# mache102/HashNeRF-pytorch

Measured on AMD Instinct MI355X. Metric: training rays/sec (fwd+bwd) on chair; PSNR@5k iters, higher is better.
Workload: dtype fp32 (MLP GEMMs split-bf16 MFMA: 3 parts fwd, 2 parts grads); 1 GPU; chair 1xMI355X N_rand=4096 64+128 L16 F2 T19 finest512 (BASELINE configs[1]); rays_per_gpu=4096, global_batch=4096, samples_per_ray=64+128, log2_hashmap_size=19, finest_res=512, parallelism=dp1

## Files before the change

hashnerf-pytorch_amd/_lib.py:

```python
from __future__ import annotations

import ctypes as C
import os
from typing import Optional

import torch

HERE = os.path.dirname(os.path.abspath(__file__))
LIB_PATH = os.environ.get("HN_LIB_PATH") or os.path.join(HERE, "lib", "libhashnerf_amd.so")
MAX_LEVELS = 32
ABI_VERSION = 14
RENDER_FEAT_PER_RAY = 9728
MLP_PARAMS = 9344
MLP_PACKED_FLOATS = 30208

_lib = None


class HnGrid(C.Structure):
    _fields_ = [("n_levels", C.c_int32), ("n_features", C.c_int32),
                ("log2_hashmap_size", C.c_int32), ("reserved", C.c_int32),
                ("box_min", C.c_float * 3), ("box_max", C.c_float * 3),
                ("grid_size", (C.c_float * 3) * MAX_LEVELS)]

# ... 28 lines not shown
                ("rgb0", _P), ("depth0", _P), ("acc0", _P), ("sparsity0", _P),
                ("z_std", _P), ("z_coarse", _P), ("z_fine", _P), ("raw_c", _P), ("raw_f", _P),
                ("fine_src", _P), ("feat", _P), ("weights_packed", C.c_int32), ("skip_dead_color", C.c_int32),
                ("loss", C.POINTER(HnRenderLoss))]


class HnImageArgs(C.Structure):
    _fields_ = [("n_views", C.c_int32), ("H", C.c_int32), ("W", C.c_int32), ("pose_stride", C.c_int32),
                ("fx", C.c_float), ("fy", C.c_float), ("cx", C.c_float), ("cy", C.c_float),
                ("near", C.c_float), ("far", C.c_float), ("poses", _P), ("t_vals", _P), ("u", _P), ("table", _P),
                ("coarse", HnMlp), ("fine", HnMlp), ("rgb", _P), ("depth", _P), ("acc", _P), ("rays", _P),
                ("weights_packed", C.c_int32)]


IMAGE_VARIANTS = {"reencode": 1, "row_major": 2}


class HnRadamTensor(C.Structure):
    _fields_ = [("p", _P), ("g", _P), ("m", _P), ("v", _P), ("n", C.c_int64),
                ("beta1", C.c_float), ("beta2", C.c_float), ("one_minus_beta1", C.c_float),
                ("one_minus_beta2", C.c_float), ("eps", C.c_float), ("neg_wd_lr", C.c_float),
                ("neg_step_lr", C.c_float), ("mode", C.c_int32), ("has_wd", C.c_int32),
                ("reserved", C.c_int32)]


class HnRaySampler(C.Structure):
    _fields_ = [("H", C.c_int32), ("W", C.c_int32), ("crop_y0", C.c_int32), ("crop_x0", C.c_int32),
                ("crop_h", C.c_int32), ("crop_w", C.c_int32), ("fx", C.c_float), ("fy", C.c_float),
                ("cx", C.c_float), ("cy", C.c_float), ("near", C.c_float), ("far", C.c_float),
                ("seed", C.c_uint64)]
# ... 70 lines not shown
    "hn_sample_pool": (C.c_int32, [C.POINTER(HnRayPool), _P, _P, _P, C.c_int64, C.c_int64, _P, _P, _P]),
    "hn_sample_pool_ordered": (C.c_int32, [C.POINTER(HnRayPool), _P, _P, _P, C.c_int64, C.c_int64,
                                           C.POINTER(C.c_float), C.POINTER(C.c_float), _P, _P, _P, C.c_uint64,
                                           C.POINTER(HnUniformDraw), C.c_int32, _P]),
    "hn_blender_images": (C.c_int32, [_P, C.c_int64, C.c_int32, C.c_int32, C.c_int32, C.c_int32, _P, _P]),
    "hn_loss_fwd": (C.c_int32, [_P, _P, _P, _P, _P, C.c_int64, _P, C.c_int32, C.c_float, C.c_float,
                                C.c_float, _P, _P]),
    "hn_loss_bwd": (C.c_int32, [_P, _P, _P, C.c_int64, C.c_int32, C.c_float, C.c_float, C.c_float, _P,
                                _P, _P, _P, _P, _P, _P]),
    "hn_loss_fwd_bwd": (C.c_int32, [_P, _P, _P, _P, _P, C.c_int64, _P, C.c_int32, C.c_float, C.c_float,
                                    C.c_float, _P, _P, _P, _P, _P, _P, _P, _P]),
    "hn_render_workspace_bytes": (C.c_size_t, [C.POINTER(HnRenderCfg), C.c_int64]),
    "hn_render_scatter_mode": (C.c_int32, [C.POINTER(HnRenderCfg), C.c_int64]),
    "hn_render_fwd": (C.c_int32, [C.POINTER(HnRenderCfg), C.POINTER(HnRenderFwdArgs), _P,
                                  C.c_size_t, _P]),
    "hn_render_bwd": (C.c_int32, [C.POINTER(HnRenderCfg), C.POINTER(HnRenderBwdArgs), _P,
                                  C.c_size_t, _P]),
    "hn_render_image_workspace_bytes": (C.c_size_t, [C.POINTER(HnRenderCfg)]),
    "hn_render_image": (C.c_int32, [C.POINTER(HnRenderCfg), C.POINTER(HnImageArgs), _P, C.c_size_t, _P]),
    "hn_render_image_variant": (C.c_int32, [C.POINTER(HnRenderCfg), C.POINTER(HnImageArgs), C.c_int32, _P,
                                            C.c_size_t, _P]),
    "hn_render_bins": (C.c_int32, [C.POINTER(HnRenderCfg), C.c_int64, C.POINTER(C.c_int32)]),
    "hn_render_bwd_owner": (C.c_int32, [C.POINTER(HnRenderCfg), C.POINTER(HnRenderBwdArgs), _P,
                                        C.c_size_t, C.c_int32, C.c_int32, _P]),
}


def lib():
    global _lib
    if _lib is None:
# ... 85 lines not shown
```

hashnerf-pytorch_amd/csrc/hn_mlp.h:

```cpp
#pragma once
#include "hn_common.h"

namespace hn {

constexpr int kSplitF = 3;
constexpr int kSplitB = 2;
enum : int { R_F0, R_F1, R_F2G, R_F2S, R_F3, R_F4, R_B4, R_B3, R_B2G, R_B2S, R_B1, R_B0, R_N };
constexpr int kRegKS[R_N] = {16, 32, 8, 8, 32, 32, 4, 32, 32, 32, 8, 32};
constexpr int kRegOB[R_N] = {2, 1, 2, 2, 2, 1, 2, 2, 1, 1, 2, 1};
constexpr int kSplitFC = kSplitF;
constexpr int reg_ns(int r) {
  return kRegKS[r] % 8 ? 0 : (r < R_F2G ? kSplitF : (r < R_B4 ? kSplitFC : kSplitB));
}
constexpr int reg_gpo(int r) { return reg_ns(r) ? reg_ns(r) * kRegKS[r] / 8 : kRegKS[r] / 4; }
constexpr int reg_off(int r) {
  int o = 0;
  for (int i = 0; i < r; ++i) o += kRegOB[i] * reg_gpo(i) * 256;
  return o;
}
enum : int {
  G_F0 = reg_off(R_F0), G_F1 = reg_off(R_F1), G_F2G = reg_off(R_F2G), G_F2S = reg_off(R_F2S),
  G_F3 = reg_off(R_F3), G_F4 = reg_off(R_F4), G_B4 = reg_off(R_B4), G_B3 = reg_off(R_B3),
  G_B2G = reg_off(R_B2G), G_B2S = reg_off(R_B2S), G_B1 = reg_off(R_B1), G_B0 = reg_off(R_B0),
  G_END = reg_off(R_N)
};
static_assert(G_END <= HN_MLP_PACKED_FLOATS, "packed size");

enum : int { W_S0 = 0, W_S1 = 2048, W_C0 = 3072, W_C1 = 5056, W_C2 = 9152, W_END = 9344 };
static_assert(W_END == HN_MLP_PARAMS, "param count");

struct FragGlobal {
  static constexpr bool kRing = false;
  const float* P;
  HN_DEV f32x4 operator()(int off, int lane) const { return frag_load(P, off, lane); }
};
struct FwdChunk {
  int r, ob, c;
};
constexpr FwdChunk kFwdSeq[] = {
    {R_F0, 0, 0}, {R_F0, 0, 1}, {R_F0, 1, 0}, {R_F0, 1, 1}, {R_F1, 0, 0}, {R_F1, 0, 1}, {R_F1, 0, 2},
    {R_F1, 0, 3}, {R_F2G, 0, 0}, {R_F2G, 1, 0}, {R_F3, 0, 0}, {R_F3, 0, 1}, {R_F3, 0, 2}, {R_F3, 0, 3},
    {R_F3, 1, 0}, {R_F3, 1, 1}, {R_F3, 1, 2}, {R_F3, 1, 3}, {R_F4, 0, 0}, {R_F4, 0, 1}, {R_F4, 0, 2},
    {R_F4, 0, 3}};
constexpr int kFwdSeqN = sizeof(kFwdSeq) / sizeof(kFwdSeq[0]);
constexpr int fwd_chunk_off(const FwdChunk& q) { return reg_off(q.r) + (q.ob * reg_gpo(q.r) + reg_ns(q.r) * q.c) * 256; }
constexpr int fwd_next_off(int r, int ob, int c) {
  for (int i = 0; i < kFwdSeqN; ++i)
    if (kFwdSeq[i].r == r && kFwdSeq[i].ob == ob && kFwdSeq[i].c == c) return fwd_chunk_off(kFwdSeq[(i + 1) % kFwdSeqN]);
  return -1;
}
struct FragRing {
  static constexpr bool kRing = true;
  const float* P;
  float* slot;
  HN_DEV f32x4 operator()(int off, int lane) const { return frag_load(P, off, lane); }
};
HN_DEV void ring_fill(const float* P, float* slot, int off, int lane) {
  int so = off * 4;
  asm volatile("" : "+s"(so));
  const __amdgpu_buffer_rsrc_t rs =
      __builtin_amdgcn_make_buffer_rsrc(const_cast<float*>(opaque_ptr(P)), (short)0, 0x7fffffff, 0x00020000);
#pragma unroll
  for (int q = 0; q < 3; ++q)
    __builtin_amdgcn_raw_ptr_buffer_load_lds(rs, (__attribute__((address_space(3))) void*)(slot + 256 * q), 16,
                                             lane * 16, so + 1024 * q, 0, 0);
}
HN_DEV void fwd_ring_start(const float* P, float* slot, int lane) {
  ring_fill(P, slot, fwd_chunk_off(kFwdSeq[0]), lane);
}
template <int R, typename BF, typename Src>
HN_DEV f32x16 gemm_src(const Src& src, int ob, f32x16 acc, int lane, BF bval);
template <int R, typename BF>
HN_DEV f32x16 gemm(const float* __restrict__ P, int ob, f32x16 acc, int lane, BF bval) {
  return gemm_src<R>(FragGlobal{P}, ob, acc, lane, bval);
}
template <int R, typename BF, typename Src>
HN_DEV f32x16 gemm_src(const Src& src, int ob, f32x16 acc, int lane, BF bval) {
  constexpr int KS = kRegKS[R], NS = reg_ns(R), GPO = reg_gpo(R), OFF = reg_off(R);
  auto ld = [&](int g) { return src(OFF + (ob * GPO + g) * 256, lane); };
  if constexpr (NS > 0) {
#pragma unroll
    for (int c = 0; c < KS / 8; ++c) {
      SP<NS> a;
      if constexpr (Src::kRing && NS == 3) {
        asm volatile("s_waitcnt vmcnt(0)" ::: "memory");
#pragma unroll
        for (int q = 0; q < NS; ++q) a.p[q] = as_bf16x8(*reinterpret_cast<const f32x4*>(src.slot + 256 * q + 4 * lane));
        asm volatile("s_waitcnt lgkmcnt(0)" ::: "memory");
        ring_fill(src.P, src.slot, fwd_next_off(R, ob, c), lane);
      } else {
#pragma unroll
        for (int q = 0; q < NS; ++q) a.p[q] = as_bf16x8(ld(NS * c + q));
      }
      const SP<NS> b = splitn<NS>([&](int j) { return bval(8 * c + j); });
// ... 295 lines not shown
```

hashnerf-pytorch_amd/csrc/hn_render.hip:

```cpp
#include "hn_render_args.h"
#include "hn_render_fwd.h"
#include "hn_render_image.h"
#include "hn_mlp_bwd.h"
#include "hn_bwd_binned.h"
#include "hn_bwd_atomic.h"

#include <math.h>

namespace hn {

__global__ __launch_bounds__(256) void render_comp_bwd_kernel(B1K k) {
  __shared__ float lds[kFwdWaves][kSf * 5];
  const int wave = __builtin_amdgcn_readfirstlane((int)threadIdx.x >> 6);
  const int lane = threadIdx.x & 63;
  if (k.bins && blockIdx.x == 0) zero_ovf_book(k);
  if (k.lout && blockIdx.x == 0) {
    loss_fwd_block<64 * kFwdWaves>(k.lrgb, k.lrgb0, k.ltarget, k.lsp, k.lsp0, k.B, k.ltv, k.n_tv, k.lworld,
                                   k.lsparse_w, k.ltv_w, k.lout);
    return;
  }
  const int64_t w = (int64_t)(blockIdx.x - (k.lout ? 1 : 0)) * kFwdWaves + wave;
  __shared__ unsigned long long cmask[kFwdWaves / 2];
  const bool active = w < 2 * k.B;
  uint32_t nzf = 0u;
// ... 236 lines not shown
  return bwd_plan(cfg, n_rays).bytes();
}

extern "C" int32_t hn_render_scatter_mode(const hn_render_cfg* cfg, int64_t n_rays) {
  return bwd_mode(cfg, n_rays) == kModeSplit ? 2 : 1;
}

extern "C" int32_t hn_device_faults(int32_t* faults, int32_t clear) {
  if (!faults) return HN_E_NULL;
  int32_t st = hip_status(hipMemcpyFromSymbol(faults, HIP_SYMBOL(g_hn_fault), sizeof(int32_t)));
  if (st || !clear || *faults == 0) return st;
  const int32_t zero = 0;
  return hip_status(hipMemcpyToSymbol(HIP_SYMBOL(g_hn_fault), &zero, sizeof(int32_t)));
}

extern "C" int32_t hn_render_fwd(const hn_render_cfg* cfg, const hn_render_fwd_args* a,
                                 void* workspace, size_t ws_bytes, void* stream) {
  int32_t st = check_cfg(cfg);
  if (st) return st;
  if (!a) return HN_E_NULL;
  if (a->n_rays < 0) return HN_E_SHAPE;
  if (a->n_rays == 0) return HN_OK;
  if (!a->rays || !a->t_vals || !a->u || !a->table || !mlp_ok(a->coarse) || !mlp_ok(a->fine))
    return HN_E_NULL;
  if (cfg->perturb && !a->t_rand) return HN_E_NULL;
  if (!a->rgb || !a->depth || !a->acc || !a->sparsity || !a->rgb0 || !a->depth0 || !a->acc0 ||
      !a->sparsity0 || !a->z_std || !a->z_coarse || !a->z_fine || !a->raw_c || !a->raw_f ||
      !a->fine_src)
    return HN_E_NULL;
  if (!workspace) return HN_E_NULL;
  const BwdPlan plan = bwd_plan(cfg, a->n_rays);
  if (ws_bytes < plan.bytes()) return HN_E_WORKSPACE;
  const bool ni64 = cfg->n_importance == kNi64;
  if (ni64 && a->feat && plan.mode != kModeSplit) return HN_E_SHAPE;
// ... 9 lines not shown
  k.perturb = cfg->perturb;
  k.B = a->n_rays;
  k.rays = a->rays; k.t_rand = a->t_rand;
  k.noise_c = a->noise_c; k.noise_f = a->noise_f;
  k.rgb = a->rgb; k.depth = a->depth; k.acc = a->acc; k.sparsity = a->sparsity;
  k.rgb0 = a->rgb0; k.depth0 = a->depth0; k.acc0 = a->acc0; k.sparsity0 = a->sparsity0;
  k.z_std = a->z_std; k.z_coarse = a->z_coarse; k.z_fine = a->z_fine;
  k.raw_c = a->raw_c; k.raw_f = a->raw_f; k.fine_src = a->fine_src; k.feat = a->feat;
  k.feat_nt = cfg->grid.log2_hashmap_size > 20;
  k.skip_dead = a->skip_dead_color != 0;
  k.ltarget = nullptr;
  k.lgm = k.lsparse = 0.f;
  k.draw = nullptr;
  k.uflags = nullptr;
  k.stamp = nullptr;
  const unsigned blocks = (unsigned)((a->n_rays + kFwdBlockWaves - 1) / kFwdBlockWaves);
  if (a->loss) {
    const WsDraw w = ws_draw(workspace, a->n_rays);
    k.ltarget = a->loss->target;
    k.lgm = (1.f / a->loss->world) / (float)(3 * a->n_rays);
    k.lsparse = 1.f * a->loss->sparse_w;
    k.draw = w.draw;
    k.uflags = w.uflags;
    k.stamp = ws_stamp(w.lmeta);
    if (ni64)
      hipLaunchKernelGGL((render_fwd_kernel<true, kNi64>), dim3(blocks), dim3(64 * kFwdBlockWaves), 0, s, k);
    else
      hipLaunchKernelGGL((render_fwd_kernel<true, kNi>), dim3(blocks), dim3(64 * kFwdBlockWaves), 0, s, k);
  } else if (ni64) {
    hipLaunchKernelGGL((render_fwd_kernel<false, kNi64>), dim3(blocks), dim3(64 * kFwdBlockWaves), 0, s, k);
  } else {
    hipLaunchKernelGGL((render_fwd_kernel<false, kNi>), dim3(blocks), dim3(64 * kFwdBlockWaves), 0, s, k);
  }
  return hip_status(hipGetLastError());
}

static size_t image_ws_floats() { return (size_t)2 * G_END + (size_t)kImgBlocks * kFwdBlockWaves * kImgSlotFloats; }

extern "C" size_t hn_render_image_workspace_bytes(const hn_render_cfg* cfg) {
  return check_image_cfg(cfg) ? 0 : image_ws_floats() * sizeof(float);
}

extern "C" int32_t hn_render_image_variant(const hn_render_cfg* cfg, const hn_image_args* a, int32_t variant,
                                           void* workspace, size_t ws_bytes, void* stream) {
  int32_t st = check_image_cfg(cfg);
  if (st) return st;
  if (!a) return HN_E_NULL;
  if (cfg->perturb) return HN_E_SHAPE;
  if (a->H <= 0 || a->W <= 0 || a->n_views < 0 || (a->pose_stride != 12 && a->pose_stride != 16)) return HN_E_SHAPE;
  if (variant < 0 || variant > (kImgReencode | kImgRowMajor)) return HN_E_SHAPE;
  if (a->n_views == 0) return HN_OK;
  if (!a->poses || !a->t_vals || !a->u || !a->table || !mlp_ok(a->coarse) || !mlp_ok(a->fine)) return HN_E_NULL;
// ... 5 lines not shown
  k.Wb = ((uint32_t)a->W + 1) / 2;
  if ((uint64_t)a->H * (uint64_t)a->W > 0x7fffffffull) return HN_E_SHAPE;
  const uint64_t groups = (variant & kImgRowMajor) ? ((uint64_t)a->n_views * a->H * a->W + 3) / 4
                                                   : (uint64_t)a->n_views * k.Hb * k.Wb;
  if (groups > 0x7fffffffull) return HN_E_SHAPE;
  hipStream_t s = (hipStream_t)stream;
  if ((st = field_args(cfg, a->t_vals, a->u, a->table, a->coarse, a->fine, a->weights_packed, workspace, s, k.f)))
    return st;
  k.variant = variant;
  k.n_views = a->n_views; k.H = a->H; k.W = a->W; k.pose_stride = a->pose_stride;
  k.groups = (uint32_t)groups;
  k.fx = a->fx; k.fy = a->fy; k.cx = a->cx; k.cy = a->cy; k.near = a->near; k.far = a->far;
  k.poses = a->poses;
  k.slots = (variant & kImgReencode) ? nullptr : (float*)workspace + 2 * (size_t)G_END;
  k.rgb = a->rgb; k.depth = a->depth; k.acc = a->acc; k.rays = a->rays;
  hipLaunchKernelGGL(render_image_kernel, dim3(kImgBlocks), dim3(64 * kFwdBlockWaves), 0, s, k);
  return hip_status(hipGetLastError());
}

extern "C" int32_t hn_render_image(const hn_render_cfg* cfg, const hn_image_args* a, void* workspace,
                                   size_t ws_bytes, void* stream) {
  return hn_render_image_variant(cfg, a, 0, workspace, ws_bytes, stream);
}

extern "C" int32_t hn_render_bins(const hn_render_cfg* cfg, int64_t n_rays, int32_t* shift) {
  if (!cfg || !shift) return 0;
  *shift = 0;
  if (check_cfg(cfg)) return 0;
  const BwdPlan plan = bwd_plan(cfg, n_rays);
  if (plan.mode != kModeSplit) return 0;
  *shift = plan.bg.shift;
// ... 271 lines not shown
```

hashnerf-pytorch_amd/csrc/hn_render_fwd.h:

```cpp
#pragma once
#include "hn_render_args.h"

#define HN_FWD_PRIO_HI() __builtin_amdgcn_s_setprio(1)
#define HN_FWD_PRIO_LO() __builtin_amdgcn_s_setprio(0)

namespace hn {

constexpr int kFZc = 0, kFZsrc = 64, kFZs = 256, kFRaw = 448, kFW = 1216, kFBins = 1280,
              kFCdf = 1344, kFC0 = 1408, kFLds = 1472;

constexpr int kFwdWavesPerSimd = 4;

constexpr int kFwdBlockWaves = kFwdWaves;


HN_DEV float coarse_z(float t, float near, float far, int lindisp) {
  return lindisp ? 1.f / (1.f / near * (1.f - t) + 1.f / far * t) : near * (1.f - t) + far * t;
}

HN_DEV void pass_start(const float* P, const float sh8[8], float* L, float* ring, int lane, bool drain) {
  c0sh_lds_store(opaque_ptr(P), sh8, L + kFC0, lane);
  lds_fence_wave();
  if (drain) asm volatile("s_waitcnt vmcnt(0)" ::: "memory");
  fwd_ring_start(P, ring, lane);
}

HN_DEV void load_twin_feat(const float* tiles, int src, int h, f32x16& feat) {
  const f32x4* t = reinterpret_cast<const f32x4*>(tiles + (size_t)(src >> 5) * 1024) + (src & 31) + 32 * h;
#pragma unroll
  for (int c = 0; c < 4; ++c) {
    const f32x4 v = t[64 * c];
    feat[4 * c] = v.x; feat[4 * c + 1] = v.y; feat[4 * c + 2] = v.z; feat[4 * c + 3] = v.w;
  }
}

template <int kNiT = kNi>
HN_DEV void importance_sort(float* L, const float* u, uint8_t* org, int lane) {
  static_assert(kNiT == kNi || kNiT == kNi64, "importance_sort: 128 or 64 importance samples");
  float* zsrc = L + kFZsrc;
  lds_fence_wave();
  sample_pdf_wave(L + kFBins, L + kFW + 1, kSc - 2, L + kFCdf, u, kNiT, zsrc + kSc, lane);
  lds_fence_wave();
  if constexpr (kNiT == kNi) {
    if (!merge_sort_z(zsrc, L + kFZs, L + kFRaw, lane, org)) rank_sort_wave(zsrc, L + kFZs, kSf, lane, org, kSc);
  } else {
    if (!merge_sort_z64(zsrc, L + kFZs, L + kFRaw, lane, org))
      rank_sort_wave(zsrc, L + kFZs, kSc + kNiT, lane, org, kSc);
  }
}

template <int kPass, class Pol, int kFineT = kSf>
HN_DEV void pass_tiles(const FieldK& f, const float* gsl, float* ring, float* L, const Ray& r, int lane, Pol& pol) {
  const int p = lane & 31, h = lane >> 5;
  for (int tau = 0; tau < (kPass ? kFineT : kSc) / 32; ++tau) {
    const float* P = opaque_ptr(kPass ? f.Pf : f.Pc);
    if constexpr (kPass && kFineT != kSf) {
      int zero = 0;
      asm volatile("" : "+s"(zero));
      gsl += zero;
    }
    const int q = 32 * tau + p;
    float pt[3];
    ray_point(r, L[(kPass ? kFZs : kFZc) + q], pt);
    f32x16 feat;
    const float* twins = kPass ? pol.twins() : nullptr;
    const int src = twins ? pol.origin(q) : 255;
    if (src >= kSc) {
      HN_FWD_PRIO_HI();
      encode_tile(f.g, gsl, f.table, pt, h, feat);
      HN_FWD_PRIO_LO();
    } else {
      load_twin_feat(twins, src, h, feat);
    }
    MlpAct a;
    f32x16 c2;
    const bool dead_skip = pol.skip_dead(kPass);
    bool stored = kPass == 0 || !dead_skip;
    if (stored) pol.save_feat(kPass, tau, lane, feat);
    mlp_fwd_tile_src<Pol::kMasks>(FragRing{P, ring}, feat, [&](int ob) { return c0sh_lds_load(L + kFC0, ob, lane); },
                                  a, c2, lane, dead_skip, [&]() {
                                    if (!stored) pol.save_feat(kPass, tau, lane, feat);
                                    stored = true;
                                  });
    const float4 o4 = make_float4(c2[0], c2[1], c2[2], a.s1[0]);
    if (stored) pol.save_masks(kPass, tau, lane, a.m);
    if (h == 0) {
      *reinterpret_cast<float4*>(L + kFRaw + 4 * q) = o4;
      pol.save_raw(kPass, q, o4);
    }
  }
}

template <bool kLoss, int kSfT>
struct TrainTiles {
// ... 22 lines not shown
    composite_fwd<N>(rawb, z, noise, S, dnorm, k.f.white != 0, wout, o, lane);
  } else {
    const float target[3] = {k.ltarget[3 * ray], k.ltarget[3 * ray + 1], k.ltarget[3 * ray + 2]};
    CompSamples<N> cs;
    composite_samples<N>(rawb, z, noise, S, dnorm, cs, lane);
    CompTotals t;
    composite_totals<N>(cs, t);
    composite_fwd_out<N>(cs, t, k.f.white != 0, wout, o, lane);
    CompGrad g;
    loss_comp_grad(g, k.lgm, k.lsparse, o.rgb[0], o.rgb[1], o.rgb[2], target);
    composite_bwd_raw<N>(cs, t, k.f.white != 0, g, nullptr, nullptr, rawb, lane);
    lds_fence_wave();
  }
}

template <bool kLoss, int kNiT>
__global__ __launch_bounds__(64 * kFwdBlockWaves)
__attribute__((amdgpu_waves_per_eu(kFwdWavesPerSimd, kFwdWavesPerSimd)))
void render_fwd_kernel(RenderK k) {
  constexpr int kSfT = kSc + kNiT;
  __shared__ __attribute__((aligned(16))) float smem[kFwdBlockWaves * kFLds + kGsLds];
  __shared__ __attribute__((aligned(16))) float fring[kFwdBlockWaves][768];
  const int wave = __builtin_amdgcn_readfirstlane((int)threadIdx.x >> 6);
  const int lane = threadIdx.x & 63;
  float* gsl = smem + kFwdBlockWaves * kFLds;
  stage_grid_sizes(k.f.g, gsl);
  __syncthreads();
  const int64_t nb = gridDim.x;
  const int64_t grp = nb % 8 == 0 ? (blockIdx.x % 8) * (nb / 8) + blockIdx.x / 8 : blockIdx.x;
  const int64_t ray = grp * kFwdBlockWaves + wave;
  if constexpr (kLoss) {
    if (blockIdx.x == 0 && threadIdx.x == 0) *k.stamp = stamp_word(k.B);
  }
  if (ray >= k.B) return;
  float* L = smem + wave * kFLds;
  float* zc = L + kFZc;
  float* zsrc = L + kFZsrc;
  float* zs = L + kFZs;
  float* rawb = L + kFRaw;
  float* wts = L + kFW;
  Ray r;
  load_ray(k.rays, ray, r);
  float sh8[8];

  auto zlin = [&](int i) { return coarse_z(k.f.tvals[i], r.near, r.far, k.f.lindisp); };
// ... 1 lines not shown
  if (k.perturb) {
    const float zm = lane > 0 ? zlin(lane - 1) : z;
    const float zp = lane < kSc - 1 ? zlin(lane + 1) : z;
    const float lower = lane > 0 ? .5f * (z + zm) : z;
    const float upper = lane < kSc - 1 ? .5f * (zp + z) : z;
    z = lower + (upper - lower) * k.t_rand[ray * kSc + lane];
  }
  zc[lane] = z;
  zsrc[lane] = z;
  k.z_coarse[ray * kSc + lane] = z;
  ray_sh(r, lane >> 5, sh8);
  lds_fence_wave();

  uint8_t* srcl = reinterpret_cast<uint8_t*>(zsrc);
  TrainTiles<kLoss, kSfT> pol{k, ray, srcl};
  pass_start(k.f.Pc, sh8, L, fring[wave], lane, false);
  pass_tiles<0>(k.f, gsl, fring[wave], L, r, lane, pol);
  lds_fence_wave();
  CompOut co;
  composite_pass<kLoss, kSc / 64>(k, ray, rawb, zc, k.noise_c ? k.noise_c + ray * kSc : nullptr, kSc, r.dnorm, wts,
                                  co, lane);
  if (lane == 0) {
#pragma unroll
    for (int c = 0; c < 3; ++c) k.rgb0[3 * ray + c] = co.rgb[c];
    k.depth0[ray] = co.depth;
    k.acc0[ray] = co.acc;
    k.sparsity0[ray] = co.entropy;
  }
  unsigned long long cmask = 0ull;
  if constexpr (kLoss) {
    const uint32_t nzu = draw_store_marks(rawb, k.draw + (size_t)ray * (kSc + kSf) * 4, kSc, lane);
    if (lane == 0) k.uflags[kMarkB * ray] = (uint8_t)nzu;
// ... 6 lines not shown
    if constexpr (kNiT == kNi) {
      const float s0 = zsrc[kSc + lane], s1 = zsrc[kSc + 64 + lane];
      const double mean = wave_sum((double)s0 + (double)s1) / kNi;
      const double d0 = (double)s0 - mean, d1 = (double)s1 - mean;
      const double var = wave_sum(d0 * d0 + d1 * d1) / kNi;
      if (lane == 0) k.z_std[ray] = (float)sqrt(var);
    } else {
      const double s0 = (double)zsrc[kSc + lane];
      const double d0 = s0 - wave_sum(s0) / kNiT;
      const double var = wave_sum(d0 * d0) / kNiT;
      if (lane == 0) k.z_std[ray] = (float)sqrt(var);
    }
  }
  for (int i = lane; i < kSfT; i += 64) k.z_fine[ray * kSfT + i] = zs[i];

  pass_start(k.f.Pf, sh8, L, fring[wave], lane, true);
  if constexpr (kLoss) {
    for (int i = lane; i < kSfT; i += 64) srcl[i] = k.fine_src[ray * kSfT + i];
    lds_fence_wave();
  }
  pass_tiles<1, TrainTiles<kLoss, kSfT>, kSfT>(k.f, gsl, fring[wave], L, r, lane, pol);
  lds_fence_wave();
  CompOut fo;
  composite_pass<kLoss, kSfT / 64>(k, ray, rawb, zs, k.noise_f ? k.noise_f + ray * kSfT : nullptr, kSfT, r.dnorm,
                                   nullptr, fo, lane);
  if (lane == 0) {
#pragma unroll
    for (int c = 0; c < 3; ++c) k.rgb[3 * ray + c] = fo.rgb[c];
    k.depth[ray] = fo.depth;
    k.acc[ray] = fo.acc;
    k.sparsity[ray] = fo.entropy;
  }
  if constexpr (kLoss) {
    const uint32_t nzf = draw_store_marks(rawb, k.draw + ((size_t)ray * (kSc + kSf) + kSc) * 4, kSfT, lane);
    const uint32_t su = scatter_marks<kSfT>(rawb, srcl, cmask, lane);
    if (lane == 0) store_fine_marks(k.uflags, ray, nzf, su);
// ... 6 lines not shown
```

hashnerf-pytorch_amd/csrc/hn_render_image.h:

```cpp
#pragma once
#include "hn_render_fwd.h"
#include "hn_sampler.h"

namespace hn {

constexpr int kImgBlocks = 1024;
constexpr int kImgSlotFloats = 2 * 1024;
static_assert(kImgBlocks % 8 == 0, "one band of ray groups per XCD residue");
constexpr int kImgTile = 8;

enum : int { kImgReencode = 1, kImgRowMajor = 2 };

struct ImageK {
  FieldK f;
  int variant;
  int n_views, H, W, pose_stride;
  uint32_t Hb, Wb;
  uint32_t groups;
  float fx, fy, cx, cy, near, far;
  const float* poses;
  float* slots;
  float *rgb, *depth, *acc, *rays;
};

// ... 39 lines not shown
  static constexpr bool kMasks = false;
  float* slot;
  const uint8_t* srcl;
  HN_DEV const float* twins() const { return slot; }
  HN_DEV int origin(int q) const { return (int)srcl[q]; }
  HN_DEV bool skip_dead(int) const { return true; }
  HN_DEV void save_feat(int pass, int tau, int lane, const f32x16& feat) const {
    if (pass == 0 && slot) store_feat(slot, 0, tau, lane, feat, false);
  }
  HN_DEV void save_masks(int, int, int, const uint32_t (&)[3]) const {}
  HN_DEV void save_raw(int, int, const float4&) const {}
};

HN_DEV float wave_uniform(float v) { return __int_as_float(__builtin_amdgcn_readfirstlane(__float_as_int(v))); }

__global__ __launch_bounds__(64 * kFwdBlockWaves)
__attribute__((amdgpu_waves_per_eu(kFwdWavesPerSimd, kFwdWavesPerSimd)))
void render_image_kernel(ImageK k) {
  __shared__ __attribute__((aligned(16))) float smem[kFwdBlockWaves * kFLds + kGsLds + kImgPixLds];
  __shared__ __attribute__((aligned(16))) float fring[kFwdBlockWaves][768];
  const int wave = __builtin_amdgcn_readfirstlane((int)threadIdx.x >> 6);
  const int lane0 = threadIdx.x & 63;
  float* gsl = smem + kFwdBlockWaves * kFLds;
  const float* pixl = gsl + kGsLds;
  stage_grid_sizes(k.f.g, gsl);
  if (threadIdx.x == 64) {
    ImagePix x;
    x.fx = k.fx; x.fy = k.fy; x.cx = k.cx; x.cy = k.cy; x.near = k.near; x.far = k.far;
    x.H = k.H; x.W = k.W; x.pose_stride = k.pose_stride; x.variant = k.variant;
    x.Hb = k.Hb; x.Wb = k.Wb;
    x.poses = k.poses;
    x.rgb = k.rgb; x.depth = k.depth; x.acc = k.acc; x.rays = k.rays;
    const uint32_t* w = reinterpret_cast<const uint32_t*>(&x);
#pragma unroll
    for (int i = 0; i < (int)(sizeof(ImagePix) / 4); ++i) gsl[kGsLds + i] = __uint_as_float(w[i]);
  }
  __syncthreads();
  float* slot = k.slots ? k.slots + ((size_t)blockIdx.x * kFwdBlockWaves + wave) * kImgSlotFloats : nullptr;

  {
    const int lane = lane0;
    float* L = smem + wave * kFLds;
    const float z = coarse_z(k.f.tvals[lane], k.near, k.far, k.f.lindisp);
    L[kFZc + lane] = z;
    L[kFZsrc + lane] = z;
    lds_fence_wave();
    if (lane < kSc - 1) L[kFBins + lane] = .5f * (L[kFZc + lane + 1] + L[kFZc + lane]);
    lds_fence_wave();
  }

  const uint32_t nbx = gridDim.x / 8, xcd = blockIdx.x % 8;
  const uint32_t lo = (uint32_t)((uint64_t)k.groups * xcd / 8), hi = (uint32_t)((uint64_t)k.groups * (xcd + 1) / 8);
  for (uint32_t grp = lo + blockIdx.x / 8; grp < hi; grp += nbx) {
    int lane = lane0, woff = wave * kFLds;
    asm volatile("" : "+v"(lane), "+s"(woff));
    float* L = smem + woff;
    uint8_t* srcl = reinterpret_cast<uint8_t*>(L + kFW);
    int64_t ray;
    Ray r;
    {
      ImagePix x;
      image_pix_load(pixl, x);
      int px, py;
      uint32_t view;
      if (x.variant & kImgRowMajor) {
        const uint32_t per_view = (uint32_t)x.H * (uint32_t)x.W;
        ray = (int64_t)grp * kFwdBlockWaves + wave;
        if (ray >= (int64_t)k.n_views * per_view) continue;
        view = (uint32_t)(ray / per_view);
        const uint32_t i = (uint32_t)(ray - (int64_t)view * per_view);
        py = (int)(i / (uint32_t)x.W);
        px = (int)(i - (uint32_t)py * (uint32_t)x.W);
      } else {
        uint32_t bx, by;
        image_group_block(x.Hb, x.Wb, grp, view, bx, by);
        px = (int)(2 * bx) + (wave & 1);
        py = (int)(2 * by) + (wave >> 1);
        if (px >= x.W || py >= x.H) continue;
        ray = ((int64_t)view * x.H + py) * x.W + px;
      }
      float v[11];
      pixel_ray(x.fx, x.fy, x.cx, x.cy, x.near, x.far, x.poses + (size_t)view * x.pose_stride, px, py, v);
// ... 39 lines not shown
```

hashnerf-pytorch_amd/functional.py:

```python
from __future__ import annotations

import ctypes as C
import os
import weakref
from typing import Optional, Sequence

import torch

from . import _lib as L


class KernelTimer:

    def __init__(self):
        self.events = {}
        self.enabled = False
        self.names = None
        self.every = 1
        self.calls = {}

    def begin(self, name):
        if not self.enabled or (self.names is not None and name not in self.names):
            return None
        c = self.calls.get(name, 0)
# ... 12 lines not shown
        self.events.setdefault(name, []).append((start, e))

    def mean_ms(self, name):
        ev = self.events.get(name, [])
        return sum(s.elapsed_time(e) for s, e in ev) / max(len(ev), 1)

    def reset(self):
        self.events = {}
        self.calls = {}


TIMER = KernelTimer()

DEBUG_KEEP = False
LAST = {}
CHECK_FAULTS = os.environ.get("HN_CHECK_FAULTS", "0") == "1"


def _ws(nbytes: int, device) -> torch.Tensor:
    return torch.empty(max(int(nbytes), 16), dtype=torch.uint8, device=device)


def _ws_size(wsb) -> int:
    return wsb.numel() * wsb.element_size()


def _caller_ws(who: str, wsb, nbytes: int, dev):
    if wsb is None:
        return _ws(nbytes, dev), nbytes
    if _ws_size(wsb) < nbytes or not wsb.is_contiguous() or wsb.device != dev:
# ... 128 lines not shown

class RenderState:
    __slots__ = ("cfg", "rays", "noise_c", "noise_f", "table", "ws", "z_c", "z_f", "raw_c", "raw_f",
                 "fine_src", "feat", "wsb", "nbytes", "bwd_args", "skip_dead", "prepass_done", "__weakref__")


def _fine_counts(cfg):
    ni = int(cfg.n_importance)
    return ni, int(cfg.n_samples) + ni


_PREPASS_ON_WS = {}


def render_fwd(cfg, rays, t_vals, t_rand, u, noise_c, noise_f, table, ws, keep_feat, wsb=None,
               weights_packed=False, skip_dead_color=False, loss=None):
    L.require_device(rays, t_vals, t_rand, u, noise_c, noise_f, table, *ws)
    rays, t_vals, t_rand, u, noise_c, noise_f = (L.contig(t) for t in (rays, t_vals, t_rand, u,
                                                                      noise_c, noise_f))
    ws = [w.contiguous() for w in ws]
    B = rays.shape[0]
    dev = rays.device
    ni, nf = _fine_counts(cfg)
    for name, t, w in (("u", u, ni), ("noise_f", noise_f, nf)):
        if t is not None and (t.numel() != B * w or (t.dim() and t.shape[-1] != w)):
            raise ValueError(f"hashnerf_amd.render_fwd: {name} must be [{B}, {w}] for n_importance = {ni}, "
                             f"got {tuple(t.shape)}")
    if keep_feat and ni != 128 and L.lib().hn_render_scatter_mode(cfg, B) != 2:
        raise ValueError("hashnerf_amd.render_fwd: n_importance = 64 trains on the binned backward only "
                         "(hn_render_scatter_mode != 2 for this configuration)")
    e = lambda *s: torch.empty(s, dtype=torch.float32, device=dev)
# ... 18 lines not shown
    a.weights_packed = 1 if weights_packed else 0
    a.skip_dead_color = 1 if skip_dead_color else 0
    la = None
    if loss is not None:
        if not keep_feat:
            raise ValueError("hashnerf_amd.render_fwd: loss= is for a forward whose backward follows (keep_feat)")
        target = L.contig(loss["target"])
        L.require_device(target)
        if tuple(target.shape) != (B, 3):
            raise ValueError(f"hashnerf_amd.render_fwd: loss target must be [{B}, 3]")
        la = L.HnRenderLoss()
        la.target = target.data_ptr()
        la.world, la.sparse_w = float(loss["world"]), float(loss["sparse_w"])
        a.loss = C.pointer(la)
    t0 = TIMER.begin("render_fwd")
    L.check(L.lib().hn_render_fwd(cfg, a, L.ptr(wsb), nbytes, L.stream(dev)), "render_fwd")
    TIMER.end("render_fwd", t0)
    if DEBUG_KEEP:
        LAST.update({k: out[k] for k in ("z_coarse", "z_fine", "raw_c", "raw_f")})
    st = None
    if keep_feat:
        st = RenderState()
        st.cfg, st.rays, st.noise_c, st.noise_f, st.table, st.ws = cfg, rays, noise_c, noise_f, table, ws
        st.z_c, st.z_f, st.raw_c, st.raw_f = out["z_coarse"], out["z_fine"], out["raw_c"], out["raw_f"]
        st.fine_src, st.feat, st.wsb, st.nbytes = fine_src, feat, wsb, nbytes
        st.bwd_args = None
        st.skip_dead = bool(skip_dead_color)
        st.prepass_done = None if la is None else (target.data_ptr(), float(loss["world"]),
                                                   float(loss["sparse_w"]))
        if la is not None:
            _PREPASS_ON_WS[wsb.data_ptr()] = weakref.ref(st)
# ... 117 lines not shown
        st.prepass_done = None
    t0 = TIMER.begin("render_bwd")
    L.check(L.lib().hn_render_bwd(st.cfg, a, L.ptr(st.wsb), st.nbytes, L.stream(dev)), "render_bwd")
    TIMER.end("render_bwd", t0)
    st.bwd_args = (a, keep, step) if owner_defer else None
    if CHECK_FAULTS and not owner_defer:
        L.check_device_faults()


def render_bins(cfg, n_rays: int):
    shift = C.c_int32(0)
    n = L.lib().hn_render_bins(cfg, n_rays, C.byref(shift))
    return int(n), int(shift.value)


def render_bwd_owner(st: RenderState, bin_lo: int, bin_hi: int):
    if getattr(st, "bwd_args", None) is None:
        raise RuntimeError("hashnerf_amd.render_bwd_owner: needs a render_bwd(owner_defer=True) first")
    a = st.bwd_args[0]
    L.check(L.lib().hn_render_bwd_owner(st.cfg, a, L.ptr(st.wsb), st.nbytes, bin_lo, bin_hi,
                                        L.stream(st.rays.device)), "render_bwd_owner")
    if CHECK_FAULTS:
        L.check_device_faults()


def zeros_like_all(ts):
    n = sum(t.numel() for t in ts)
    flat = torch.zeros(n, dtype=torch.float32, device=ts[0].device)
    out, off = [], 0
    for t in ts:
# ... 443 lines not shown
```

include/hashnerf_amd.h:

```cpp
#ifndef HASHNERF_AMD_H
#define HASHNERF_AMD_H

#include <stddef.h>
#include <stdint.h>

#ifdef __cplusplus
extern "C" {
#endif

#define HN_ABI_VERSION 14
#define HN_MAX_LEVELS 32

enum {
  HN_OK = 0,
  HN_E_NULL = 1,
  HN_E_SHAPE = 2,
  HN_E_WORKSPACE = 3,
  HN_E_HIP = 1000
};

typedef struct hn_grid {
  int32_t n_levels;
  int32_t n_features;
  int32_t log2_hashmap_size;
// ... 211 lines not shown
int32_t hn_loss_fwd(const float* rgb, const float* rgb0, const float* target, const float* sp,
                    const float* sp0, int64_t n_rays, const float* tv, int32_t n_tv, float world,
                    float sparse_w, float tv_w, float* out, void* stream);
int32_t hn_loss_bwd(const float* rgb, const float* rgb0, const float* target, int64_t n_rays,
                    int32_t n_tv, float world, float sparse_w, float tv_w, const float* g_loss,
                    float* g_rgb, float* g_rgb0, float* g_sp, float* g_sp0, float* g_tv, void* stream);
int32_t hn_loss_fwd_bwd(const float* rgb, const float* rgb0, const float* target, const float* sp,
                        const float* sp0, int64_t n_rays, const float* tv, int32_t n_tv, float world,
                        float sparse_w, float tv_w, float* out, const float* g_loss, float* g_rgb,
                        float* g_rgb0, float* g_sp, float* g_sp0, float* g_tv, void* stream);

size_t hn_render_workspace_bytes(const hn_render_cfg* cfg, int64_t n_rays);
int32_t hn_render_scatter_mode(const hn_render_cfg* cfg, int64_t n_rays);
int32_t hn_render_fwd(const hn_render_cfg* cfg, const hn_render_fwd_args* a,
                      void* workspace, size_t ws_bytes, void* stream);
int32_t hn_render_bwd(const hn_render_cfg* cfg, const hn_render_bwd_args* a,
                      void* workspace, size_t ws_bytes, void* stream);

typedef struct hn_image_args {
  int32_t n_views, H, W;
  int32_t pose_stride;
  float fx, fy, cx, cy;
  float near, far;
  const float* poses;
  const float* t_vals;
  const float* u;
  const float* table;
  hn_mlp coarse, fine;
  float* rgb;
  float* depth; float* acc;
// ... 14 lines not shown
```

Measured before the change: 8.071 million rays/s.

## Add block-resident LDS MLP weight form for training forward kernel

Adds a second forward-render variant in which a 16-wave block cooperatively stages the early-layer packed MLP weights (coarse and fine) into shared memory once. The GEMM fragments for those layers are then read from LDS instead of each wave filling its own weight ring. It also remaps rays into per-block runs, and auto-selects this form when the ray count gives at least one block per CU. The aim is to cut redundant per-wave weight fetches and ring traffic. In exchange it uses larger blocks and shares LDS across waves, which may reduce scheduling flexibility.

```diff
diff --git a/hashnerf-pytorch_amd/_lib.py b/hashnerf-pytorch_amd/_lib.py
--- a/hashnerf-pytorch_amd/_lib.py
+++ b/hashnerf-pytorch_amd/_lib.py
@@ -66,6 +66,14 @@
 
 
 IMAGE_VARIANTS = {"reencode": 1, "row_major": 2}
+FWD_FORMS = {"auto": 0, "ring": 1, "resident": 2}
+
+
+def fwd_form(form) -> int:
+    v = FWD_FORMS.get(form, form) if isinstance(form, str) else form
+    if isinstance(v, bool) or not isinstance(v, int) or v not in FWD_FORMS.values():
+        raise ValueError(f"hashnerf_amd.render_fwd: form must be one of {sorted(FWD_FORMS)} or 0, 1, 2, got {form!r}")
+    return v
 
 
 class HnRadamTensor(C.Structure):
@@ -166,6 +174,9 @@
     "hn_render_scatter_mode": (C.c_int32, [C.POINTER(HnRenderCfg), C.c_int64]),
     "hn_render_fwd": (C.c_int32, [C.POINTER(HnRenderCfg), C.POINTER(HnRenderFwdArgs), _P,
                                   C.c_size_t, _P]),
+    "hn_render_fwd_form": (C.c_int32, [C.POINTER(HnRenderCfg), C.POINTER(HnRenderFwdArgs), C.c_int32, _P,
+                                       C.c_size_t, _P]),
+    "hn_render_fwd_pick": (C.c_int32, [C.c_int64, C.POINTER(C.c_int32)]),
     "hn_render_bwd": (C.c_int32, [C.POINTER(HnRenderCfg), C.POINTER(HnRenderBwdArgs), _P,
                                   C.c_size_t, _P]),
     "hn_render_image_workspace_bytes": (C.c_size_t, [C.POINTER(HnRenderCfg)]),
diff --git a/hashnerf-pytorch_amd/csrc/hn_mlp.h b/hashnerf-pytorch_amd/csrc/hn_mlp.h
--- a/hashnerf-pytorch_amd/csrc/hn_mlp.h
+++ b/hashnerf-pytorch_amd/csrc/hn_mlp.h
@@ -31,6 +31,7 @@
 
 struct FragGlobal {
   static constexpr bool kRing = false;
+  static constexpr int kLdsEnd = 0;
   const float* P;
   HN_DEV f32x4 operator()(int off, int lane) const { return frag_load(P, off, lane); }
 };
@@ -51,9 +52,19 @@
 }
 struct FragRing {
   static constexpr bool kRing = true;
+  static constexpr int kLdsEnd = 0;
   const float* P;
   float* slot;
   HN_DEV f32x4 operator()(int off, int lane) const { return frag_load(P, off, lane); }
+};
+constexpr int kFragResFloats = G_F2G;
+struct FragRes {
+  static constexpr bool kRing = false;
+  static constexpr int kLdsEnd = kFragResFloats;
+  const float* P;
+  const float* res;
+  HN_DEV f32x4 operator()(int off, int lane) const { return frag_load(P, off, lane); }
+  HN_DEV f32x4 lds(int off, int lane) const { return *reinterpret_cast<const f32x4*>(res + off + 4 * lane); }
 };
 HN_DEV void ring_fill(const float* P, float* slot, int off, int lane) {
   int so = off * 4;
@@ -77,7 +88,10 @@
 template <int R, typename BF, typename Src>
 HN_DEV f32x16 gemm_src(const Src& src, int ob, f32x16 acc, int lane, BF bval) {
   constexpr int KS = kRegKS[R], NS = reg_ns(R), GPO = reg_gpo(R), OFF = reg_off(R);
-  auto ld = [&](int g) { return src(OFF + (ob * GPO + g) * 256, lane); };
+  auto ld = [&](int g) {
+    if constexpr (OFF < Src::kLdsEnd) return src.lds(OFF + (ob * GPO + g) * 256, lane);
+    else return src(OFF + (ob * GPO + g) * 256, lane);
+  };
   if constexpr (NS > 0) {
 #pragma unroll
     for (int c = 0; c < KS / 8; ++c) {
diff --git a/hashnerf-pytorch_amd/csrc/hn_render.hip b/hashnerf-pytorch_amd/csrc/hn_render.hip
--- a/hashnerf-pytorch_amd/csrc/hn_render.hip
+++ b/hashnerf-pytorch_amd/csrc/hn_render.hip
@@ -6,6 +6,8 @@
 #include "hn_bwd_atomic.h"
 
 #include <math.h>
+
+#include <atomic>
 
 namespace hn {
 
@@ -274,10 +276,46 @@
   return hip_status(hipMemcpyToSymbol(HIP_SYMBOL(g_hn_fault), &zero, sizeof(int32_t)));
 }
 
+static int device_cus() {
+  static std::atomic<int> cached[64];
+  int dev = 0;
+  if (hipGetDevice(&dev) != hipSuccess || dev < 0 || dev >= 64) return 0;
+  int n = cached[dev].load(std::memory_order_relaxed);
+  if (n == 0) {
+    if (hipDeviceGetAttribute(&n, hipDeviceAttributeMultiprocessorCount, dev) != hipSuccess || n < 0) n = 0;
+    cached[dev].store(n, std::memory_order_relaxed);
+  }
+  return n;
+}
+static int fwd_pick_form(int64_t n_rays, int cus) {
+  return cus > 0 && (n_rays + kFwdResWaves - 1) / kFwdResWaves >= cus ? 2 : 1;
+}
+template <bool kLoss, int kNiT>
+static void launch_fwd(bool res, int64_t n_rays, hipStream_t s, const RenderK& k) {
+  const int bw = fwd_block_waves(res);
+  const dim3 grid((unsigned)((n_rays + bw - 1) / bw)), block(64 * bw);
+  if (res)
+    hipLaunchKernelGGL((render_fwd_kernel<kLoss, kNiT, true>), grid, block, 0, s, k);
+  else
+    hipLaunchKernelGGL((render_fwd_kernel<kLoss, kNiT, false>), grid, block, 0, s, k);
+}
+
+extern "C" int32_t hn_render_fwd_pick(int64_t n_rays, int32_t* cus) {
+  const int n = device_cus();
+  if (cus) *cus = n;
+  return fwd_pick_form(n_rays, n);
+}
+
 extern "C" int32_t hn_render_fwd(const hn_render_cfg* cfg, const hn_render_fwd_args* a,
                                  void* workspace, size_t ws_bytes, void* stream) {
+  return hn_render_fwd_form(cfg, a, 0, workspace, ws_bytes, stream);
+}
+
+extern "C" int32_t hn_render_fwd_form(const hn_render_cfg* cfg, const hn_render_fwd_args* a, int32_t form,
+                                      void* workspace, size_t ws_bytes, void* stream) {
   int32_t st = check_cfg(cfg);
   if (st) return st;
+  if (form < 0 || form > 2) return HN_E_SHAPE;
   if (!a) return HN_E_NULL;
   if (a->n_rays < 0) return HN_E_SHAPE;
   if (a->n_rays == 0) return HN_OK;
@@ -317,7 +355,7 @@
   k.draw = nullptr;
   k.uflags = nullptr;
   k.stamp = nullptr;
-  const unsigned blocks = (unsigned)((a->n_rays + kFwdBlockWaves - 1) / kFwdBlockWaves);
+  const bool res = (form ? form : fwd_pick_form(a->n_rays, device_cus())) == 2;
   if (a->loss) {
     const WsDraw w = ws_draw(workspace, a->n_rays);
     k.ltarget = a->loss->target;
@@ -327,18 +365,18 @@
     k.uflags = w.uflags;
     k.stamp = ws_stamp(w.lmeta);
     if (ni64)
-      hipLaunchKernelGGL((render_fwd_kernel<true, kNi64>), dim3(blocks), dim3(64 * kFwdBlockWaves), 0, s, k);
+      launch_fwd<true, kNi64>(res, a->n_rays, s, k);
     else
-      hipLaunchKernelGGL((render_fwd_kernel<true, kNi>), dim3(blocks), dim3(64 * kFwdBlockWaves), 0, s, k);
+      launch_fwd<true, kNi>(res, a->n_rays, s, k);
   } else if (ni64) {
-    hipLaunchKernelGGL((render_fwd_kernel<false, kNi64>), dim3(blocks), dim3(64 * kFwdBlockWaves), 0, s, k);
+    launch_fwd<false, kNi64>(res, a->n_rays, s, k);
   } else {
-    hipLaunchKernelGGL((render_fwd_kernel<false, kNi>), dim3(blocks), dim3(64 * kFwdBlockWaves), 0, s, k);
+    launch_fwd<false, kNi>(res, a->n_rays, s, k);
   }
   return hip_status(hipGetLastError());
 }
 
-static size_t image_ws_floats() { return (size_t)2 * G_END + (size_t)kImgBlocks * kFwdBlockWaves * kImgSlotFloats; }
+static size_t image_ws_floats() { return (size_t)2 * G_END + (size_t)kImgBlocks * kImgBlockWaves * kImgSlotFloats; }
 
 extern "C" size_t hn_render_image_workspace_bytes(const hn_render_cfg* cfg) {
   return check_image_cfg(cfg) ? 0 : image_ws_floats() * sizeof(float);
@@ -374,7 +412,7 @@
   k.poses = a->poses;
   k.slots = (variant & kImgReencode) ? nullptr : (float*)workspace + 2 * (size_t)G_END;
   k.rgb = a->rgb; k.depth = a->depth; k.acc = a->acc; k.rays = a->rays;
-  hipLaunchKernelGGL(render_image_kernel, dim3(kImgBlocks), dim3(64 * kFwdBlockWaves), 0, s, k);
+  hipLaunchKernelGGL(render_image_kernel, dim3(kImgBlocks), dim3(64 * kImgBlockWaves), 0, s, k);
   return hip_status(hipGetLastError());
 }
 
diff --git a/hashnerf-pytorch_amd/csrc/hn_render_fwd.h b/hashnerf-pytorch_amd/csrc/hn_render_fwd.h
--- a/hashnerf-pytorch_amd/csrc/hn_render_fwd.h
+++ b/hashnerf-pytorch_amd/csrc/hn_render_fwd.h
@@ -12,17 +12,21 @@
 constexpr int kFwdWavesPerSimd = 4;
 
 constexpr int kFwdBlockWaves = kFwdWaves;
+constexpr int kFwdResWaves = 16;
+constexpr int kFwdResRuns = 4;
+constexpr int fwd_block_waves(bool res) { return res ? kFwdResWaves : kFwdBlockWaves; }
 
 
 HN_DEV float coarse_z(float t, float near, float far, int lindisp) {
   return lindisp ? 1.f / (1.f / near * (1.f - t) + 1.f / far * t) : near * (1.f - t) + far * t;
 }
 
+template <bool kRes = false>
 HN_DEV void pass_start(const float* P, const float sh8[8], float* L, float* ring, int lane, bool drain) {
   c0sh_lds_store(opaque_ptr(P), sh8, L + kFC0, lane);
   lds_fence_wave();
   if (drain) asm volatile("s_waitcnt vmcnt(0)" ::: "memory");
-  fwd_ring_start(P, ring, lane);
+  if constexpr (!kRes) fwd_ring_start(P, ring, lane);
 }
 
 HN_DEV void load_twin_feat(const float* tiles, int src, int h, f32x16& feat) {
@@ -49,12 +53,12 @@
   }
 }
 
-template <int kPass, class Pol, int kFineT = kSf>
+template <int kPass, class Pol, int kFineT = kSf, bool kRes = false>
 HN_DEV void pass_tiles(const FieldK& f, const float* gsl, float* ring, float* L, const Ray& r, int lane, Pol& pol) {
   const int p = lane & 31, h = lane >> 5;
   for (int tau = 0; tau < (kPass ? kFineT : kSc) / 32; ++tau) {
     const float* P = opaque_ptr(kPass ? f.Pf : f.Pc);
-    if constexpr (kPass && kFineT != kSf) {
+    if constexpr (kPass && (kFineT != kSf || kRes)) {
       int zero = 0;
       asm volatile("" : "+s"(zero));
       gsl += zero;
@@ -77,7 +81,8 @@
     const bool dead_skip = pol.skip_dead(kPass);
     bool stored = kPass == 0 || !dead_skip;
     if (stored) pol.save_feat(kPass, tau, lane, feat);
-    mlp_fwd_tile_src<Pol::kMasks>(FragRing{P, ring}, feat, [&](int ob) { return c0sh_lds_load(L + kFC0, ob, lane); },
+    using Src = std::conditional_t<kRes, FragRes, FragRing>;
+    mlp_fwd_tile_src<Pol::kMasks>(Src{P, ring}, feat, [&](int ob) { return c0sh_lds_load(L + kFC0, ob, lane); },
                                   a, c2, lane, dead_skip, [&]() {
                                     if (!stored) pol.save_feat(kPass, tau, lane, feat);
                                     stored = true;
@@ -130,21 +135,41 @@
   }
 }
 
-template <bool kLoss, int kNiT>
-__global__ __launch_bounds__(64 * kFwdBlockWaves)
+template <bool kLoss, int kNiT, bool kRes = false>
+__global__ __launch_bounds__(64 * fwd_block_waves(kRes))
 __attribute__((amdgpu_waves_per_eu(kFwdWavesPerSimd, kFwdWavesPerSimd)))
 void render_fwd_kernel(RenderK k) {
   constexpr int kSfT = kSc + kNiT;
-  __shared__ __attribute__((aligned(16))) float smem[kFwdBlockWaves * kFLds + kGsLds];
-  __shared__ __attribute__((aligned(16))) float fring[kFwdBlockWaves][768];
+  constexpr int kBW = fwd_block_waves(kRes);
+  __shared__ __attribute__((aligned(16))) float smem[kBW * kFLds + kGsLds];
+  static_assert(2 * kFragResFloats % (4 * kFwdResWaves) == 0, "a whole dwordx4 share per wave");
+  __shared__ __attribute__((aligned(16))) float fring[kBW][kRes ? 2 * kFragResFloats / kFwdResWaves : 768];
   const int wave = __builtin_amdgcn_readfirstlane((int)threadIdx.x >> 6);
   const int lane = threadIdx.x & 63;
-  float* gsl = smem + kFwdBlockWaves * kFLds;
+  float* gsl = smem + kBW * kFLds;
   stage_grid_sizes(k.f.g, gsl);
+  if constexpr (kRes) {
+    constexpr int kN4 = kFragResFloats / 4;
+    const f32x4* srcc = reinterpret_cast<const f32x4*>(k.f.Pc);
+    const f32x4* srcf = reinterpret_cast<const f32x4*>(k.f.Pf);
+    f32x4* dst = reinterpret_cast<f32x4*>(&fring[0][0]);
+#pragma unroll
+    for (int i = 0; i < (2 * kN4 + 64 * kBW - 1) / (64 * kBW); ++i) {
+      const int j = i * 64 * kBW + (int)threadIdx.x;
+      if (j < 2 * kN4) dst[j] = j < kN4 ? srcc[j] : srcf[j - kN4];
+    }
+  }
   __syncthreads();
   const int64_t nb = gridDim.x;
   const int64_t grp = nb % 8 == 0 ? (blockIdx.x % 8) * (nb / 8) + blockIdx.x / 8 : blockIdx.x;
-  const int64_t ray = grp * kFwdBlockWaves + wave;
+  int64_t ray = grp * kBW + wave;
+  if constexpr (kRes) {
+    constexpr int kW = kBW / kFwdResRuns;
+    const int s = wave / kW;
+    const int64_t run = nb % 8 == 0 ? (blockIdx.x % 8) * (nb / 8 * kFwdResRuns) + s * (nb / 8) + blockIdx.x / 8
+                                    : s * nb + blockIdx.x;
+    ray = run * kW + wave % kW;
+  }
   if constexpr (kLoss) {
     if (blockIdx.x == 0 && threadIdx.x == 0) *k.stamp = stamp_word(k.B);
   }
@@ -176,8 +201,10 @@
 
   uint8_t* srcl = reinterpret_cast<uint8_t*>(zsrc);
   TrainTiles<kLoss, kSfT> pol{k, ray, srcl};
-  pass_start(k.f.Pc, sh8, L, fring[wave], lane, false);
-  pass_tiles<0>(k.f, gsl, fring[wave], L, r, lane, pol);
+  float* srcc = kRes ? &fring[0][0] : fring[wave];
+  float* srcf = kRes ? &fring[0][0] + kFragResFloats : fring[wave];
+  pass_start<kRes>(k.f.Pc, sh8, L, srcc, lane, false);
+  pass_tiles<0, TrainTiles<kLoss, kSfT>, kSf, kRes>(k.f, gsl, srcc, L, r, lane, pol);
   lds_fence_wave();
   CompOut co;
   composite_pass<kLoss, kSc / 64>(k, ray, rawb, zc, k.noise_c ? k.noise_c + ray * kSc : nullptr, kSc, r.dnorm, wts,
@@ -214,12 +241,12 @@
   }
   for (int i = lane; i < kSfT; i += 64) k.z_fine[ray * kSfT + i] = zs[i];
 
-  pass_start(k.f.Pf, sh8, L, fring[wave], lane, true);
+  pass_start<kRes>(k.f.Pf, sh8, L, srcf, lane, true);
   if constexpr (kLoss) {
     for (int i = lane; i < kSfT; i += 64) srcl[i] = k.fine_src[ray * kSfT + i];
     lds_fence_wave();
   }
-  pass_tiles<1, TrainTiles<kLoss, kSfT>, kSfT>(k.f, gsl, fring[wave], L, r, lane, pol);
+  pass_tiles<1, TrainTiles<kLoss, kSfT>, kSfT, kRes>(k.f, gsl, srcf, L, r, lane, pol);
   lds_fence_wave();
   CompOut fo;
   composite_pass<kLoss, kSfT / 64>(k, ray, rawb, zs, k.noise_f ? k.noise_f + ray * kSfT : nullptr, kSfT, r.dnorm,
diff --git a/hashnerf-pytorch_amd/csrc/hn_render_image.h b/hashnerf-pytorch_amd/csrc/hn_render_image.h
--- a/hashnerf-pytorch_amd/csrc/hn_render_image.h
+++ b/hashnerf-pytorch_amd/csrc/hn_render_image.h
@@ -5,6 +5,7 @@
 namespace hn {
 
 constexpr int kImgBlocks = 1024;
+constexpr int kImgBlockWaves = kFwdWaves;
 constexpr int kImgSlotFloats = 2 * 1024;
 static_assert(kImgBlocks % 8 == 0, "one band of ray groups per XCD residue");
 constexpr int kImgTile = 8;
@@ -77,14 +78,14 @@
 
 HN_DEV float wave_uniform(float v) { return __int_as_float(__builtin_amdgcn_readfirstlane(__float_as_int(v))); }
 
-__global__ __launch_bounds__(64 * kFwdBlockWaves)
+__global__ __launch_bounds__(64 * kImgBlockWaves)
 __attribute__((amdgpu_waves_per_eu(kFwdWavesPerSimd, kFwdWavesPerSimd)))
 void render_image_kernel(ImageK k) {
-  __shared__ __attribute__((aligned(16))) float smem[kFwdBlockWaves * kFLds + kGsLds + kImgPixLds];
-  __shared__ __attribute__((aligned(16))) float fring[kFwdBlockWaves][768];
+  __shared__ __attribute__((aligned(16))) float smem[kImgBlockWaves * kFLds + kGsLds + kImgPixLds];
+  __shared__ __attribute__((aligned(16))) float fring[kImgBlockWaves][768];
   const int wave = __builtin_amdgcn_readfirstlane((int)threadIdx.x >> 6);
   const int lane0 = threadIdx.x & 63;
-  float* gsl = smem + kFwdBlockWaves * kFLds;
+  float* gsl = smem + kImgBlockWaves * kFLds;
   const float* pixl = gsl + kGsLds;
   stage_grid_sizes(k.f.g, gsl);
   if (threadIdx.x == 64) {
@@ -99,7 +100,7 @@
     for (int i = 0; i < (int)(sizeof(ImagePix) / 4); ++i) gsl[kGsLds + i] = __uint_as_float(w[i]);
   }
   __syncthreads();
-  float* slot = k.slots ? k.slots + ((size_t)blockIdx.x * kFwdBlockWaves + wave) * kImgSlotFloats : nullptr;
+  float* slot = k.slots ? k.slots + ((size_t)blockIdx.x * kImgBlockWaves + wave) * kImgSlotFloats : nullptr;
 
   {
     const int lane = lane0;
@@ -128,7 +129,7 @@
       uint32_t view;
       if (x.variant & kImgRowMajor) {
         const uint32_t per_view = (uint32_t)x.H * (uint32_t)x.W;
-        ray = (int64_t)grp * kFwdBlockWaves + wave;
+        ray = (int64_t)grp * kImgBlockWaves + wave;
         if (ray >= (int64_t)k.n_views * per_view) continue;
         view = (uint32_t)(ray / per_view);
         const uint32_t i = (uint32_t)(ray - (int64_t)view * per_view);
diff --git a/hashnerf-pytorch_amd/functional.py b/hashnerf-pytorch_amd/functional.py
--- a/hashnerf-pytorch_amd/functional.py
+++ b/hashnerf-pytorch_amd/functional.py
@@ -50,6 +50,7 @@
 
 DEBUG_KEEP = False
 LAST = {}
+FWD_FORM = "auto"
 CHECK_FAULTS = os.environ.get("HN_CHECK_FAULTS", "0") == "1"
 
 
@@ -208,7 +209,8 @@
 
 
 def render_fwd(cfg, rays, t_vals, t_rand, u, noise_c, noise_f, table, ws, keep_feat, wsb=None,
-               weights_packed=False, skip_dead_color=False, loss=None):
+               weights_packed=False, skip_dead_color=False, loss=None, form=None):
+    form = L.fwd_form(FWD_FORM if form is None else form)
     L.require_device(rays, t_vals, t_rand, u, noise_c, noise_f, table, *ws)
     rays, t_vals, t_rand, u, noise_c, noise_f = (L.contig(t) for t in (rays, t_vals, t_rand, u,
                                                                       noise_c, noise_f))
@@ -257,7 +259,7 @@
         la.world, la.sparse_w = float(loss["world"]), float(loss["sparse_w"])
         a.loss = C.pointer(la)
     t0 = TIMER.begin("render_fwd")
-    L.check(L.lib().hn_render_fwd(cfg, a, L.ptr(wsb), nbytes, L.stream(dev)), "render_fwd")
+    L.check(L.lib().hn_render_fwd_form(cfg, a, form, L.ptr(wsb), nbytes, L.stream(dev)), "render_fwd")
     TIMER.end("render_fwd", t0)
     if DEBUG_KEEP:
         LAST.update({k: out[k] for k in ("z_coarse", "z_fine", "raw_c", "raw_f")})
@@ -405,6 +407,12 @@
     return int(n), int(shift.value)
 
 
+def fwd_pick(n_rays: int):
+    cus = C.c_int32(0)
+    form = L.lib().hn_render_fwd_pick(int(n_rays), C.byref(cus))
+    return {v: k for k, v in L.FWD_FORMS.items()}[int(form)], int(cus.value)
+
+
 def render_bwd_owner(st: RenderState, bin_lo: int, bin_hi: int):
     if getattr(st, "bwd_args", None) is None:
         raise RuntimeError("hashnerf_amd.render_bwd_owner: needs a render_bwd(owner_defer=True) first")
diff --git a/include/hashnerf_amd.h b/include/hashnerf_amd.h
--- a/include/hashnerf_amd.h
+++ b/include/hashnerf_amd.h
@@ -249,6 +249,9 @@
 int32_t hn_render_scatter_mode(const hn_render_cfg* cfg, int64_t n_rays);
 int32_t hn_render_fwd(const hn_render_cfg* cfg, const hn_render_fwd_args* a,
                       void* workspace, size_t ws_bytes, void* stream);
+int32_t hn_render_fwd_form(const hn_render_cfg* cfg, const hn_render_fwd_args* a, int32_t form,
+                           void* workspace, size_t ws_bytes, void* stream);
+int32_t hn_render_fwd_pick(int64_t n_rays, int32_t* cus);
 int32_t hn_render_bwd(const hn_render_cfg* cfg, const hn_render_bwd_args* a,
                       void* workspace, size_t ws_bytes, void* stream);
 
```

New measurement: 8.298 million rays/s, median of 6. +2.8%, better.
